# HiKapok/X-Detector

Hardware: AMD Instinct MI355X
Metric: images/sec at 480x480 Light-Head R-CNN, 1/2/4/8 MI355X + backbone MFMA util% (higher is better)
Workload: dtype f16x3 (split-precision f16 MFMA, f32 accumulate, f32 activations); 1 GPU; Full Light-Head R-CNN (Xception backbone + RPN + GPU proposals/NMS + PSROIAlign + light head + per-class NMS), 300 proposals, 480x480; batch_per_gpu=256, global_batch=256, image_size=480, concurrent_sub_batches=2, cross_terms=f16, input=whitened f32 [B,3,480,480] resident in HBM, parallelism=image-sharded dp1, weights=seeded random init (no checkpoint exists), graph_replay=True

## Files before the change

### x-detector_amd/csrc/common.h

```cpp
#pragma once
#include <hip/hip_runtime.h>
#include "../../include/xdet.h"
#include "conv_params.h"
#include "workspace.h"
#include <atomic>
#include <cstdint>
#include <cstdio>
#include <string>
#include <vector>

namespace xdet {

void set_last_error(const std::string& s);
int hip_fail(hipError_t e, const char* what, const char* file, int line);

#define XDET_HIP(expr)                                                          \
  do {                                                                          \
    hipError_t _e = (expr);                                                     \
    if (_e != hipSuccess) return ::xdet::hip_fail(_e, #expr, __FILE__, __LINE__); \
  } while (0)

#define XDET_LAUNCH_CHECK() XDET_HIP(hipGetLastError())

#define XDET_REQUIRE(cond, msg)                                   \
  do {                                                            \
    if (!(cond)) {                                                \
      ::xdet::set_last_error(std::string("invalid argument: ") + (msg)); \
      return XDET_ERR_INVALID_ARG;                        \
    }                                                             \
  } while (0)

#define XDET_TRY(expr)            \
  do {                            \
    int _rc = (expr);             \
    if (_rc != 0) return _rc;     \
  } while (0)

struct DeviceOnce {
  std::atomic<unsigned long long> done{0};
};
static inline int ensure_dynamic_lds(DeviceOnce& once, const void* kern, int bytes) {
  int dev = 0;
  XDET_HIP(hipGetDevice(&dev));
  const unsigned long long bit = 1ull << (dev & 63);
  if (once.done.load(std::memory_order_acquire) & bit) return XDET_OK;
  XDET_HIP(hipFuncSetAttribute(kern, hipFuncAttributeMaxDynamicSharedMemorySize, bytes));
  once.done.fetch_or(bit, std::memory_order_release);
  return XDET_OK;
}

static inline int round_up(int x, int m) { return (x + m - 1) / m * m; }
static inline int64_t cdiv(int64_t a, int64_t b) { return (a + b - 1) / b; }

int launch_conv_mfma_f32(const ConvParams& p, bool small_cin, int n_tile, hipStream_t s);
int launch_conv_mfma_split(const ConvParams& p, bool small_cin, int n_tile, int nsplit, hipStream_t s);
int launch_conv_mfma_dma(const ConvParams& p, int n_tile, int nsplit, hipStream_t s);
bool conv_dma_fold_applicable(const ConvParams& p, int n_tile, int nsplit);
int launch_conv_mfma_dma_fold(const ConvParams& p, hipStream_t s);
int64_t conv_ksplit_tiles(int64_t M, int cout_pad, int n_tile);
bool conv_ksplit_supported(int kh, int kw, int64_t n_pix_in, int ld_in, int cin_p, int cout_pad);
int launch_conv_mfma_ksplit(const ConvParams& p, int n_tile, int nsplit, int mode, int64_t scratch_tiles, hipStream_t s);
enum { PREC_F32 = 0, PREC_F16X3 = 1, PREC_F16 = 2 };

int launch_nchw_to_nhwc4(const float* in, float* out, int N, int C, int H, int W, int ldo, hipStream_t s);
int launch_depthwise3x3(const float* in, const float* w9c, float* out, int N, int H, int W, int C, int ld,
                        int dil, int relu_in, hipStream_t s);
int launch_maxpool3x3s2_add(const float* in, const float* res, float* out, int N, int H, int W, int C, int ld,
                            int Ho, int Wo, int pad_t, int pad_l, hipStream_t s);
int launch_maxpool3x3s2_bn_planes(const float* in, const float* scale, const float* shift, unsigned short* hi, unsigned short* lo,
                                  int N, int H, int W, int C, int ld, int Ho, int Wo, int pad_t, int pad_l, float mul,
                                  hipStream_t s, unsigned short* hi2 = nullptr, unsigned short* lo2 = nullptr, int c32_2 = 0,
                                  float mul2 = 1.f);
int launch_bn_relu(const float* in, const float* scale, const float* shift, float* out, unsigned short* hi, unsigned short* lo,
                   int64_t npix, int ld, float mul, hipStream_t s);
int launch_maxpool_v3s2_add(const float* in_hpooled, const float* res, float* out, int N, int H, int Wo, int C, int ld,
                            int Ho, int pad_t, hipStream_t s, unsigned short* sub_hi = nullptr, unsigned short* sub_lo = nullptr,
                            float sub_mul = 1.f);
int launch_range_check(const float* x, int N, size_t per_image, float limit, int* bad_per_image, hipStream_t s,
                       int groups = 1, size_t group_elems = 0, int relu = 0);
int launch_range_check_planes(const unsigned short* hi, int N, int64_t pix_per_image, int ld, int* bad_per_image,
                              hipStream_t s, int groups = 1, int64_t group_pix = 0);
int launch_relu_copy(const float* in, float* out, int64_t n, hipStream_t s);
int launch_stem_conv3x3s2(const float* in_nchw, const float* w27x32, const float* scale, const float* shift,
                          unsigned short* hi, unsigned short* lo, int N, int S, hipStream_t s);
int launch_split_f32(const float* in, unsigned short* hi, unsigned short* lo, int64_t n_pix, int ld, int relu,
                     hipStream_t s, float mul = 1.f, int x8 = 0, int x8_exp = 0);
int launch_planes_copy_blocks(const unsigned short* shi, const unsigned short* slo, unsigned short* dhi, unsigned short* dlo,
                              int64_t n_pix, int ld_src, int c32_dst, float r, hipStream_t s);
int launch_split_f32_subsample2(const float* in, unsigned short* hi, unsigned short* lo, int N, int H, int W, int ld,
                                hipStream_t s, const float* scale = nullptr, const float* shift = nullptr, float mul = 1.f,
                                int c32_dst = 0);
int launch_absmax_planes(const unsigned short* hi, int64_t n_halves, unsigned* out, hipStream_t s);
int launch_absmax_f32(const float* x, int64_t n, int relu, unsigned* out, hipStream_t s);
int launch_depthwise3x3_split(const float* in, const float* w9c, unsigned short* hi, unsigned short* lo, int N,
                              int H, int W, int C, int ld, int dil, int relu_in, hipStream_t s, int x8 = 0, int x8_exp = 0);

bool spectral_supported(int F);
int spectral_points(int F);
void spectral_tables(int F, std::vector<float>* fwd, std::vector<float>* inv);
void spectral_weights(const float* w, int T, int cin, int cout, int cin_ld, int cout_ld, int F, std::vector<float>* out);
int launch_dft_fwd(const float* in, int F, int ld, int axis, int N, int m_pad, const float* tab, unsigned short* hi,
                   unsigned short* lo, hipStream_t s);
int launch_dft_inv(const float* Y, int F, int ldn, int C_ld, int N, int m_pad, const float* tab, const float* scale,
                   const float* shift, int relu, float* out, int ldo, int axis, hipStream_t s);

bool sepconv_fused_supported(int cin_ld, int cout_pad, int dil);
int launch_sepconv_fused(const float* in, const float* w9c, const unsigned short* wt_hi_blocked,
                         const unsigned short* wt_lo_blocked, const float* scale, const float* shift, float* out, int N,
                         int H, int W, int ld, int ldo, int cout_pad, int relu_in, int relu_out, hipStream_t s,
                         int pool_pad_l = -1);

bool conv3x3_patch_supported(int kh, int kw, int cin, int cout_pad, int stride, int dil, int pad_mode);
int launch_conv3x3_patch(const unsigned short* in_hi, const unsigned short* in_lo, const unsigned short* wt_hi_blocked,
                         const unsigned short* wt_lo_blocked, const float* scale, const float* shift, float* out, int N, int H,
                         int W, int ldo, int relu, hipStream_t s);

bool resnet_stem7x7_supported(int kh, int kw, int cin, int cout, int stride, int pad_mode, int pad, int S);
int launch_resnet_stem7x7(const float* img_nchw, const unsigned short* wt_hi, const unsigned short* wt_lo, const float* scale,
                          const float* shift, float* out, int N, int S, hipStream_t s);

bool resnet_preconv_supported(int cin, int cmid, int64_t M);
int launch_resnet_preconv(const float* x, const float* pre_sc, const float* pre_sh, const unsigned short* w_hi,
                          const unsigned short* w_lo, const float* sc, const float* sh, unsigned short* out_hi,
                          unsigned short* out_lo, int64_t M, int cin, int cmid, hipStream_t s);

struct BneckLaunch {
  const float* x;
  const float *pre_sc, *pre_sh;
  const unsigned short *wa_hi, *wa_lo, *wb_hi, *wb_lo, *wc_hi, *wc_lo;
  const float *sc_a, *sh_a, *sc_b, *sh_b, *sc_c, *sh_c;
  const float *pl_sc, *pl_sh;
  float* out;
  unsigned short *out_hi, *out_lo;
  int H, W, cin, cmid, cout;
};
bool resnet_bneck_supported(int cin, int cmid, int cout, int H, int W, int N);
int launch_resnet_bneck(const BneckLaunch& a, int N, hipStream_t s);

int launch_preprocess_eval(const unsigned char* img, int H, int W, float* out_chw, int S, hipStream_t s);
int launch_preprocess_batch(const unsigned char* packed, int64_t packed_bytes, const int64_t* offsets,
                            const int* image_shapes, int N, int S, int mode, float* out_nchw, float* bbox_img,
                            hipStream_t s);

size_t preprocess_train_workspace_bytes(int N, int G);
int launch_preprocess_train(const unsigned char* packed, int64_t packed_bytes, const int64_t* offsets,
                            const int* image_shapes, const int* glabels, const float* gbboxes, const int* n_gt,
                            const int* image_ids, int N, int G, int S, unsigned seed, float* out_nchw, int* out_glabels,
                            float* out_gbboxes, int* out_n_gt, void* records, void* workspace, hipStream_t s);

int launch_psroialign(const float* feat, const float* rois, float* pooled, int32_t* index, int N, int C, int H,
                      int W, int R, int gw, int gh, int use_max, int layout, int ldc, int out_ld,
                      int rois_are_corners, hipStream_t s);
int launch_psroialign_grad(const float* rois, const float* grad_pooled, const int32_t* pooled_index, float* grad_out,
                           int N, int C, int H, int W, int R, int gw, int gh, int use_max, int layout, int ldc,
                           hipStream_t s);
int launch_psroialign_grad_ordered(const float* rois, const float* grad_pooled, int ld_grad, const int32_t* pooled_index,
                                   int ld_index, float* grad_out, int N, int C, int H, int W, int R, int gw, int gh,
                                   int use_max, int layout, int ldc, int corners, hipStream_t s);
int psroi_nhwc_scratch(const float* feat, int N, int C, int H, int W, hipStream_t s, float** scratch);

int launch_rotated_psroialign(const float* feat, const float* rois, const int32_t* orders, float* pooled,
                              int32_t* index, int N, int C, int H, int W, int R, int gw, int gh, int use_max,
                              int layout, int ldc, hipStream_t s);
int launch_rotated_psroialign_grad(const float* rois, const int32_t* orders, const float* grad_pooled,
                                   const int32_t* pooled_index, float* grad_out, int N, int C, int H, int W, int R,
                                   int gw, int gh, int use_max, int layout, int ldc, hipStream_t s);

struct ProposalWorkspace {
  unsigned long long* keys;
  float* cboxes;
  int* ranks;
  int* counts;
  float* sboxes;
  float* sscores;
  unsigned long long* cand;
  int* hist;
  int* bad;
  int* tbin;
  int* kept;
  unsigned* nms_ctl;
  unsigned long long* nms_sup;
// ... 23 lines not shown
```

### x-detector_amd/csrc/conv_mfma_dma.hip

```cpp
#include "common.h"
#include "conv_epilogue.h"
#include <cstdlib>
#include <cstring>
#include <type_traits>

namespace xdet {

#if CD_PROBE_LEVEL == 1
unsigned long long* g_conv_dma_probe = nullptr;
int g_conv_dma_probe_no_walk = 0;
#endif

typedef float f32x16 __attribute__((ext_vector_type(16)));
typedef _Float16 f16x8 __attribute__((ext_vector_type(8)));
typedef int x8frag __attribute__((ext_vector_type(8)));
typedef int x8half __attribute__((ext_vector_type(4)));
typedef unsigned short u16;

#define XDET_GLDS16(gptr, lptr)                                                                        \
  __builtin_amdgcn_global_load_lds((const __attribute__((address_space(1))) void*)(gptr),              \
                                   (__attribute__((address_space(3))) void*)(lptr), 16, 0, 0)

#ifndef CD_PROBE_LEVEL
#define CD_PROBE_LEVEL 0
#endif
#if CD_PROBE_LEVEL == 1
#define CD_PROBE_PARAM , unsigned long long* dbg
#define CD_PROBE_ARG , g_conv_dma_probe
#define CD_STAMP(vblk, slot)                                                      \
  do {                                                                            \
    if (dbg && threadIdx.x == 0) {                                                \
      dbg[((size_t)(vblk) * 5 + (slot)) * 2] = __builtin_amdgcn_s_memrealtime();  \
      dbg[((size_t)(vblk) * 5 + (slot)) * 2 + 1] = __builtin_amdgcn_s_memtime();  \
    }                                                                             \
  } while (0)
#define CD_STAMP_DRAINED(vblk, slot)                        \
  do {                                                      \
    asm volatile("s_waitcnt vmcnt(0)" ::: "memory");        \
    CD_STAMP(vblk, slot);                                   \
  } while (0)
#else
#define CD_PROBE_PARAM
#define CD_PROBE_ARG
#define CD_STAMP(vblk, slot) do {} while (0)
#define CD_STAMP_DRAINED(vblk, slot) do {} while (0)
#endif

constexpr int conv_dma_lds_bytes(int bm, int bn, int waves_m, int waves_n, bool walk) {
  const int stage = (2 * bm + 2 * bn) * 32 * 2;
  const int staging = waves_m * waves_n * 32 * (bn / waves_n + 4) * 4;
  return walk && stage + staging > 2 * stage ? stage + staging : 2 * stage;
}

template <int BM, int BN, int WAVES_M, int WAVES_N, int NSPLIT, int NSTAGE, bool PW = false, bool FOLD = false, bool X8 = false,
          bool GBUF = false, bool WALK = false>
__global__ __launch_bounds__(64 * WAVES_M * WAVES_N) void conv_dma_f16_kernel(ConvParams p_in, int nvb CD_PROBE_PARAM) {
  static_assert(NSTAGE == 2, "two LDS stages");
  static_assert(!(GBUF && PW), "GBUF is the buffer form of the NON-pointwise layers");
  static_assert(!X8 || (PW && NSPLIT == 3 && !FOLD), "x8: pointwise f16x3 layers only");
  static_assert(!WALK || ((PW || GBUF) && !FOLD), "the tile walk: the buffer forms (their weights are aimed per tile through a resource)");
  constexpr int NW = WAVES_M * WAVES_N;
  constexpr int WM = BM / WAVES_M, WN = BN / WAVES_N;
  constexpr int TM = WM / 32, TN = WN / 32;
  constexpr int A_IT = BM / (16 * NW);
  constexpr int B_IT = BN / (16 * NW);
  static_assert(A_IT >= 1 && B_IT >= 1, "tile too small for the wave count");
  constexpr int ROWB = 32;
  constexpr int STAGE = (2 * BM + 2 * BN) * ROWB;
  constexpr int EP_OFF = WALK ? STAGE : 0;
  constexpr int EP_BYTES = conv_dma_lds_bytes(BM, BN, WAVES_M, WAVES_N, WALK) - EP_OFF * 2;
  static_assert(conv_dma_lds_bytes(BM, BN, WAVES_M, WAVES_N, WALK) <= 160 * 1024, "stages + epilogue staging must fit a CU's LDS");

  extern __shared__ __attribute__((aligned(16))) u16 smem16[];

  const int tid = threadIdx.x;
  const int lane = tid & 63;
  const int wave = __builtin_amdgcn_readfirstlane(tid >> 6);
  const int wm = wave / WAVES_N, wn = wave % WAVES_N;
  const int nby = p_in.Cout_pad / BN;
  ConvParams p = p_in;
  auto tile_of = [&](int vb, int& tm0, int& tn0, int& tg) -> bool {
    const int slot = vb >> 3;
    if (p_in.group_rows) {
      const int mt = p_in.group_rows / BM;
      const int tpg = mt * nby;
      const int g = (slot / tpg) * 8 + (vb & 7);
      const int w = slot - (slot / tpg) * tpg;
      if ((int64_t)g * p_in.group_rows >= p_in.M) return false;
      if (p_in.group_live_rows && (w / nby) * BM >= p_in.group_live_rows) return false;
      tm0 = (g * mt + w / nby) * BM;
      tn0 = (w % nby) * BN;
      tg = g;
    } else {
      const int bx = (slot / nby) * 8 + (vb & 7);
      if (bx * BM >= p_in.M) return false;
      tm0 = bx * BM;
      tn0 = (slot % nby) * BN;
      tg = 0;
    }
    return true;
  };
  int vb = blockIdx.x;
  int m0, n0, grp;
  if constexpr (WALK) {
    while (vb < nvb && !tile_of(vb, m0, n0, grp)) vb += gridDim.x;
    if (vb >= nvb) return;
  } else {
    if (!tile_of(vb, m0, n0, grp)) return;
  }
  if (!WALK && p_in.group_rows) {
    p.wt_hi = p_in.wt_hi + (size_t)grp * p_in.group_wt_stride;
    p.wt_lo = p_in.wt_lo ? p_in.wt_lo + (size_t)grp * p_in.group_wt_stride : nullptr;
    p.scale = p_in.scale + (size_t)grp * p_in.Cout_pad;
    p.shift = p_in.shift + (size_t)grp * p_in.Cout_pad;
  }
  CD_STAMP(vb, 0);

  int iy0[A_IT], ix0[A_IT], pbase[A_IT], achunk[A_IT];
  size_t boff[B_IT];
  const int nk = p.Kp / 32;
  const int ntaps = p.KH * p.KW;
  const unsigned c32n = (unsigned)(p.ldi >> 5);

  __amdgpu_buffer_rsrc_t r_ah, r_al, r_bh, r_bl;
  unsigned a_vo[A_IT], b_vo[B_IT];
  int g_cc = 0, g_ky = 0, g_kx = 0, g_tap = 0;
  if (PW || GBUF) {
    const unsigned a_bytes = GBUF ? (unsigned)(((size_t)(((size_t)p.N * p.H * p.W + 15) >> 4) * c32n) << 10)
                                  : (unsigned)(((size_t)((p.M + 15) >> 4) * c32n) << 10);
    r_ah = __builtin_amdgcn_make_buffer_rsrc(const_cast<u16*>(p.in_hi), 0, (int)a_bytes, 0x00020000);
    r_al = __builtin_amdgcn_make_buffer_rsrc(const_cast<u16*>(NSPLIT > 1 ? p.in_lo : p.in_hi), 0, (int)a_bytes, 0x00020000);
  }
  auto aim = [&](int ln, int tm0, int tn0, int tg) {
    const int lr = ln >> 2;
    const int pos = ln & 3;
#pragma unroll
    for (int q = 0; q < A_IT; ++q) {
      const int rt = (wave * A_IT + q) * 16 + lr;
      achunk[q] = (pos ^ ((rt >> 2) & 3)) * 8;
      const int m = tm0 + rt;
      if (!PW) {
        if (m < p.M) {
          int hw = p.Ho * p.Wo, wo = p.Wo;
          if (WALK) asm volatile("" : "+s"(hw), "+s"(wo));
          const int n = m / hw;
          const int rem = m - n * hw;
          const int oy = rem / wo;
          const int ox = rem - oy * wo;
          iy0[q] = oy * p.stride - p.pad_t;
          ix0[q] = ox * p.stride - p.pad_l;
          pbase[q] = n * p.H * p.W;
        } else {
          iy0[q] = -(1 << 20);
          ix0[q] = 0;
          pbase[q] = 0;
        }
      } else {
        a_vo[q] = m < p.M ? (((unsigned)(m >> 4) * c32n) << 10) + (unsigned)((((m & 15) << 5) + achunk[q]) * 2) : 0xffffffffu;
      }
    }
#pragma unroll
    for (int q = 0; q < B_IT; ++q) {
      const int rt = (wave * B_IT + q) * 16 + lr;
      boff[q] = (size_t)(tn0 + rt) * 32 + (pos ^ ((rt >> 2) & 3)) * 8;
      if (PW || GBUF) b_vo[q] = (unsigned)(boff[q] * 2);
    }
    if (PW || GBUF) {
      const size_t wo = WALK ? (size_t)tg * p_in.group_wt_stride : 0;
      const unsigned b_bytes = (unsigned)((size_t)nk * p.Cout_pad * 64);
      r_bh = __builtin_amdgcn_make_buffer_rsrc(const_cast<u16*>(p.wt_hi + wo), 0, (int)b_bytes, 0x00020000);
      r_bl = __builtin_amdgcn_make_buffer_rsrc(const_cast<u16*>((NSPLIT > 1 ? p.wt_lo : p.wt_hi) + wo), 0, (int)b_bytes, 0x00020000);
    }
// ... 515 lines not shown
        }
      }
#pragma unroll
      for (int ks = 0; ks < 2; ++ks) {
        if (NSPLIT > 1) {
#pragma unroll
          for (int j = 0; j < TN; ++j) acc[0][j] = __builtin_amdgcn_mfma_f32_32x32x16_f16(al[ks], bh[ks][j], acc[0][j], 0, 0, 0);
#pragma unroll
          for (int j = 0; j < TN; ++j) acc[0][j] = __builtin_amdgcn_mfma_f32_32x32x16_f16(ah[ks], bl[ks][j], acc[0][j], 0, 0, 0);
        }
#pragma unroll
        for (int j = 0; j < TN; ++j) acc[0][j] = __builtin_amdgcn_mfma_f32_32x32x16_f16(ah[ks], bh[ks][j], acc[0][j], 0, 0, 0);
      }
    }
    ring = ring + PAIR >= NSTAGE ? ring + PAIR - NSTAGE : ring + PAIR;
  }
  asm volatile("s_waitcnt vmcnt(0)" ::: "memory");
  if (m0 + BM <= p.M) conv_epilogue_full<32, 32 * TN, 1, TN, NW, NSTAGE * STAGE * 2>(p, acc, smem16, wave, lane, WT ? (wave >> 1) : wave, WT ? (wave & 1) : 0, m0, n0);
  else conv_epilogue<32, 32 * TN, 1, TN, NW, NSTAGE * STAGE * 2>(p, acc, smem16, wave, lane, WT ? (wave >> 1) : wave, WT ? (wave & 1) : 0, m0, n0);
}

static bool pw_eligible(const ConvParams& p) {
  if (p.KH != 1 || p.KW != 1 || p.stride != 1 || p.pad_t != 0 || p.pad_l != 0 || p.H != p.Ho || p.W != p.Wo) return false;
  const size_t a_bytes = ((size_t)((p.M + 15) >> 4) * (size_t)(p.ldi >> 5)) << 10;
  const size_t b_bytes = (size_t)(p.Kp / 32) * p.Cout_pad * 64;
  return a_bytes < ((size_t)1 << 32) && b_bytes < ((size_t)1 << 32) && p.Cin_p == p.Kp;
}

template <int NSPLIT, bool PW = false, bool W8 = false, bool H64 = false>
static int launch_deep(const ConvParams& p, hipStream_t s) {
  if (!PW && pw_eligible(p)) return launch_deep<NSPLIT, true, W8, H64>(p, s);
  if constexpr (!W8 && !H64 && NSPLIT == 3) {
    if (!p.group_rows && cdiv(p.M, 128) * (p.Cout_pad / 64) <= 128) return launch_deep<NSPLIT, PW, false, true>(p, s);
    return launch_deep<NSPLIT, PW, true>(p, s);
  }
  constexpr int BM = H64 ? 64 : 128;
  constexpr size_t lds = (size_t)6 * (2 * BM + 2 * 64) * 32 * sizeof(u16);
  auto kern = conv_dma_deep_kernel<NSPLIT, PW, W8, H64>;
  static DeviceOnce once;
  XDET_TRY(ensure_dynamic_lds(once, reinterpret_cast<const void*>(kern), (int)lds));
  dim3 grid((unsigned)(cdiv(cdiv(p.M, BM), 8) * 8 * (p.Cout_pad / 64)));
  if (p.group_rows) {
    const int64_t groups = p.M / p.group_rows, tpg = (int64_t)(p.group_rows / BM) * (p.Cout_pad / 64);
    grid = dim3((unsigned)(cdiv(groups, 8) * 8 * tpg));
  }
  hipLaunchKernelGGL(kern, grid, dim3(W8 ? 512 : 256), lds, s, p);
  XDET_LAUNCH_CHECK();
  return XDET_OK;
}

static bool gbuf_eligible(const ConvParams& p) {
  if (p.group_rows != 0) return false;
  const size_t a_bytes = ((((size_t)p.N * p.H * p.W + 15) >> 4) * (size_t)(p.ldi >> 5)) << 10;
  const size_t b_bytes = (size_t)(p.Kp / 32) * p.Cout_pad * 64;
  return a_bytes < ((size_t)1 << 32) && b_bytes < ((size_t)1 << 32) && p.Kp == p.Cin_p * p.KH * p.KW;
}

static int device_cu_count(int* n_out) {
  static std::atomic<int> cus[64];
  int dev = 0;
  XDET_HIP(hipGetDevice(&dev));
  int n = cus[dev & 63].load(std::memory_order_acquire);
  if (n <= 0) {
    XDET_HIP(hipDeviceGetAttribute(&n, hipDeviceAttributeMultiprocessorCount, dev));
    cus[dev & 63].store(n, std::memory_order_release);
  }
  *n_out = n;
  return XDET_OK;
}

template <int BM, int BN, int WAVES_M, int WAVES_N, int NSPLIT, int NSTAGE = 2, bool PW = false, bool X8 = false, bool GBUF = false>
static int launch_d(const ConvParams& p, hipStream_t s) {
  if (!PW && pw_eligible(p)) return launch_d<BM, BN, WAVES_M, WAVES_N, NSPLIT, NSTAGE, true>(p, s);
  if constexpr (PW && !X8 && NSPLIT == 3) {
    if (p.x8) return launch_d<BM, BN, WAVES_M, WAVES_N, NSPLIT, NSTAGE, true, true>(p, s);
  }
  XDET_REQUIRE(X8 || !p.x8, "conv(dma): x8 planes need a pointwise f16x3 layer below 4 GiB");
  constexpr size_t lds = conv_dma_lds_bytes(BM, BN, WAVES_M, WAVES_N, false);
  if constexpr (!PW && !X8 && !GBUF && BM == 256 && BN == 256) {
    if (gbuf_eligible(p)) return launch_d<BM, BN, WAVES_M, WAVES_N, NSPLIT, NSTAGE, false, false, true>(p, s);
  }
  int64_t nvb = cdiv(cdiv(p.M, BM), 8) * 8 * (p.Cout_pad / BN);
  if (p.group_rows) {
    const int64_t groups = p.M / p.group_rows, tpg = (int64_t)(p.group_rows / BM) * (p.Cout_pad / BN);
    nvb = cdiv(groups, 8) * 8 * tpg;
  }
  if constexpr (BM == 256 && BN == 256 && (PW || GBUF)) {
    int cus = 0;
    XDET_TRY(device_cu_count(&cus));
    const int64_t wgs = cus / 8 * 8;
    bool walk = wgs >= 8 && nvb > wgs;
#if CD_PROBE_LEVEL == 1
    if (g_conv_dma_probe_no_walk) walk = false;
#endif
    if (walk) {
      constexpr size_t lds_w = conv_dma_lds_bytes(BM, BN, WAVES_M, WAVES_N, true);
      auto kern_w = conv_dma_f16_kernel<BM, BN, WAVES_M, WAVES_N, NSPLIT, NSTAGE, PW, false, X8, GBUF, true>;
      static DeviceOnce once_w;
      XDET_TRY(ensure_dynamic_lds(once_w, reinterpret_cast<const void*>(kern_w), (int)lds_w));
      hipLaunchKernelGGL(kern_w, dim3((unsigned)wgs), dim3(64 * WAVES_M * WAVES_N), lds_w, s, p, (int)nvb CD_PROBE_ARG);
      XDET_LAUNCH_CHECK();
      return XDET_OK;
    }
  }
  auto kern = conv_dma_f16_kernel<BM, BN, WAVES_M, WAVES_N, NSPLIT, NSTAGE, PW, false, X8, GBUF>;
  static DeviceOnce once;
  XDET_TRY(ensure_dynamic_lds(once, reinterpret_cast<const void*>(kern), (int)lds));
  hipLaunchKernelGGL(kern, dim3((unsigned)nvb), dim3(64 * WAVES_M * WAVES_N), lds, s, p, (int)nvb CD_PROBE_ARG);
  XDET_LAUNCH_CHECK();
  return XDET_OK;
}

bool conv_dma_fold_applicable(const ConvParams& p, int n_tile, int nsplit) {
  return n_tile == 128 && nsplit == 3 && p.group_rows == 0 && p.ksplit > 1 && cdiv(p.M, 256) * (p.Cout_pad / 128) >= 170;
}
int launch_conv_mfma_dma_fold(const ConvParams& p, hipStream_t s) {
  constexpr size_t lds = (size_t)2 * (2 * 256 + 2 * 128) * 32 * sizeof(u16);
  auto kern = conv_dma_f16_kernel<256, 128, 4, 2, 3, 2, false, true>;
  static DeviceOnce once;
  XDET_TRY(ensure_dynamic_lds(once, reinterpret_cast<const void*>(kern), (int)lds));
  dim3 grid((unsigned)(cdiv(cdiv(p.M, 256), 8) * 8 * (p.Cout_pad / 128)));
  hipLaunchKernelGGL(kern, grid, dim3(512), lds, s, p, (int)grid.x CD_PROBE_ARG);
  XDET_LAUNCH_CHECK();
  return XDET_OK;
}

int launch_conv_mfma_dma(const ConvParams& p_in, int n_tile, int nsplit, hipStream_t s) {
  ConvParams p = p_in;
  p.skip_dead = 1;
  XDET_REQUIRE(p.Kp % 32 == 0 && p.Cin_p % 32 == 0 && p.ldi >= p.Cin_p && p.ldi % 8 == 0,
               "conv(dma): channel counts must be padded to 32");
  XDET_REQUIRE(p.Cout_pad % n_tile == 0, "conv(dma): Cout_pad must be a multiple of the N tile");
  XDET_REQUIRE(p.in_hi && (nsplit == 1 || p.in_lo) && p.wt_hi && (nsplit == 1 || p.wt_lo) && p.zeros,
               "conv(dma): split planes missing");
  if (p.M <= 0) return XDET_OK;
  if (n_tile == 128 && nsplit == 3) {
    const int64_t b256 = cdiv(p.M, 256) * (p.Cout_pad / 256);
    const int nk = p.Kp / 32;
    int tile = 0;
    const bool full_rounds = b256 >= 240 && (b256 % 256 == 0 || b256 % 256 >= 240);
    if (p.Cout_pad % 256 == 0 && (b256 >= 512 || full_rounds || (b256 >= 200 && nk >= 40))) tile = 2;
    if (p.group_rows && p.group_rows % 256 != 0) tile = 0;
    if (tile == 2) return launch_d<256, 256, 2, 4, 3>(p, s);
  }
  if (n_tile == 128 && nsplit == 3 && !p.group_rows && !p.x8) {
    const int64_t b128 = cdiv(p.M, 128) * (p.Cout_pad / 128);
    if (b128 > 128 && b128 <= 256 && p.Kp / 32 >= 16 && p.Kp == p.Cin_p * p.KH * p.KW && p.ldi % 32 == 0 &&
        conv_ksplit_supported(p.KH, p.KW, (int64_t)p.N * p.H * p.W, p.ldi, p.Cin_p, p.Cout_pad)) {
      ConvParams q = p;
      q.ksplit = 1;
      q.ks_partial = nullptr;
      return launch_conv_mfma_ksplit(q, 128, 3, 2, 0, s);
    }
  }
  if (n_tile == 128 && nsplit == 3 && p.group_rows && p.group_rows % 64 == 0 && !p.x8) {
    const int live = p.group_live_rows ? p.group_live_rows : p.group_rows;
    const int64_t groups = p.M / p.group_rows, wgs = groups * cdiv(live, 64) * (p.Cout_pad / 64);
    if (live <= 64 && wgs <= 768) return launch_deep<3, false, false, true>(p, s);
  }
  if (n_tile == 128) {
    const int64_t b128 = cdiv(p.M, 128) * (p.Cout_pad / 128);
    if (nsplit == 3 && b128 <= 128 && (!p.group_rows || p.group_rows % 128 == 0)) {
      return p.x8 ? launch_d<128, 64, 4, 1, 3>(p, s) : launch_deep<3>(p, s);
    }
    return nsplit == 1 ? launch_d<128, 128, 2, 2, 1>(p, s) : launch_d<128, 128, 2, 2, 3>(p, s);
  }
  if (n_tile == 64) return nsplit == 1 ? launch_d<128, 64, 4, 1, 1>(p, s) : launch_d<128, 64, 4, 1, 3>(p, s);
  set_last_error("conv(dma): unsupported N tile");
// ... 5 lines not shown
```

### x-detector_amd/csrc/layers.h

```cpp
#pragma once
#include "common.h"
#include "device_mem.h"

#include <algorithm>
#include <cmath>
#include <cstring>
#include <vector>

namespace xdet {

struct Pow2Scaled {
  std::vector<float> host;
  float* dev = nullptr;
  int upload(int e, size_t n = 0) const {
    std::vector<float> v(std::max(n, host.size()), 0.f);
    for (size_t i = 0; i < host.size(); ++i) v[i] = ldexpf(host[i], e);
    XDET_HIP(hipMemcpy(dev, v.data(), v.size() * sizeof(float), hipMemcpyHostToDevice));
    return XDET_OK;
  }
};

extern int g_default_precision;

__host__ __device__ static inline unsigned short f32_to_f16_rne(float f) {
// ... 198 lines not shown
          hi[gc * kp + k] = h;
          if (precision == PREC_F16X3) lo[gc * kp + k] = f32_to_f16_rne(wv - f16_to_f32(h));
        }
        sc[gc] = ldexpf(sc[gc], -sh_k);
      }
      std::vector<float>().swap(wt);
      if (groups == 1) {
        XDET_TRY(d_wt_hi.upload(hi.data(), hi.size()));
        if (precision == PREC_F16X3) XDET_TRY(d_wt_lo.upload(lo.data(), lo.size()));
      }
      if (!small_cin) {
        std::vector<unsigned short> blk(hi.size());
        auto kblock = [&](const std::vector<unsigned short>& src) {
          for (size_t g = 0; g < G; ++g)
            for (int co = 0; co < cout_pad; ++co) {
              const unsigned short* r = &src[(g * cout_pad + co) * kp];
              for (int k = 0; k < kp; ++k) blk[g * mat + ((size_t)(k >> 5) * cout_pad + co) * 32 + (k & 31)] = r[k];
            }
        };
        kblock(hi);
        XDET_TRY(d_wt_hi_b.upload(blk.data(), blk.size()));
        if (precision == PREC_F16X3) {
          kblock(lo);
          XDET_TRY(d_wt_lo_b.upload(blk.data(), blk.size()));
          if (kh == 1 && kw == 1 && stride == 1 && groups == 1) {
            unsigned char* b8 = reinterpret_cast<unsigned char*>(blk.data());
            for (int co = 0; co < cout_pad; ++co)
              for (int k = 0; k < kp; ++k) {
                unsigned char* rec = b8 + ((size_t)(k >> 5) * cout_pad + co) * 64;
                rec[k & 31] = f32_to_e4m3(std::ldexp(f16_to_f32(lo[(size_t)co * kp + k]), 9));
                rec[32 + (k & 31)] = f32_to_e4m3(std::ldexp(f16_to_f32(hi[(size_t)co * kp + k]), -2));
              }
            XDET_TRY(d_wt_x8_b.upload(blk.data(), blk.size()));
          }
        }
      }
    }
    XDET_TRY(d_scale.upload(sc.data(), sc.size()));
    XDET_TRY(d_shift.upload(sh.data(), sh.size()));
    in_scale.host = sc;
    in_scale.dev = d_scale;
    return XDET_OK;
  }

  void out_shape(int H, int W, int* Ho, int* Wo, int* pt, int* pl) const {
    if (pad_mode == 1) {
      same_pad(H, kh, stride, dil, pt, Ho);
      same_pad(W, kw, stride, dil, pl, Wo);
    } else {
      *pt = pad_mode == 2 ? pad_t : 0;
      *pl = pad_mode == 2 ? pad_l : 0;
      const int tot_h = pad_mode == 2 ? (kh - 1) * dil : 0, tot_w = pad_mode == 2 ? (kw - 1) * dil : 0;
      *Ho = (H + tot_h - ((kh - 1) * dil + 1)) / stride + 1;
      *Wo = (W + tot_w - ((kw - 1) * dil + 1)) / stride + 1;
    }
  }
  int ld_in() const { return small_cin ? 4 : round_up(cin, 32); }
  int ld_out() const { return round_up(cout, 32); }
  double flops(int H, int W) const {
    int Ho, Wo, a, b;
    out_shape(H, W, &Ho, &Wo, &a, &b);
    return 2.0 * Ho * Wo * (double)cin * cout * kh * kw;
  }

  int forward(const ConvIO& io, int N, int H, int W, int ldi, int ldo, hipStream_t s) const {
    XDET_REQUIRE(ldi == ld_in(), "conv: ld_in must be round_up(cin,32) (4 for cin<=4)");
    XDET_REQUIRE(ldo == ld_out(), "conv: ld_out must be round_up(cout,32)");
    ConvParams p;
    p.in = io.in; p.wt = d_wt; p.wt_hi = d_wt_hi; p.wt_lo = d_wt_lo; p.out = io.out; p.scale = d_scale; p.shift = d_shift; p.res = io.res;
    p.N = N; p.H = H; p.W = W; p.ldi = ldi; p.ldo = ldo; p.ldr = ldo;
    out_shape(H, W, &p.Ho, &p.Wo, &p.pad_t, &p.pad_l);
    XDET_REQUIRE(p.Ho > 0 && p.Wo > 0, "conv: empty output");
    p.Cin_p = cin_p; p.Kp = kp; p.Cout_pad = cout_pad;
    p.KH = kh; p.KW = kw; p.stride = stride; p.dil = dil;
    p.M = N * p.Ho * p.Wo;
    p.relu_in = io.relu_in; p.relu_out = relu_out;
    p.in_hi = io.in_hi; p.in_lo = io.in_lo; p.zeros = io.zeros;
    p.out_hi = precision == PREC_F32 ? nullptr : io.out_hi; p.out_lo = io.out_lo; p.planes_relu = io.planes_relu;
    p.pl_scale = io.pl_scale; p.pl_shift = io.pl_shift; p.pl_c32 = pl_c32;
    p.group_rows = 0; p.group_wt_stride = 0;
    if (groups > 1) {
      XDET_REQUIRE(io.in_hi && io.group_rows > 0 && io.group_rows % 128 == 0 && (int64_t)io.group_rows * groups == p.M,
                   "conv(grouped): M must be groups * group_rows, group_rows a multiple of 128, input as planes");
      p.group_rows = io.group_rows;
      p.group_wt_stride = (long long)cout_pad * kp;
      p.group_live_rows = io.group_live_rows;
    }
    if (precision == PREC_F32) return launch_conv_mfma_f32(p, small_cin, n_tile, s);
    if (io.in_hi) {
      XDET_REQUIRE(!small_cin && io.relu_in == 0, "conv(dma): needs >= 32 input channels and no ReLU-on-load");
      p.wt_hi = d_wt_hi_b; p.wt_lo = d_wt_lo_b;
      if (io.x8) {
        XDET_REQUIRE(d_wt_x8_b && precision == PREC_F16X3 && ksplit < 1, "conv: x8 planes need a pointwise f16x3 layer without a split-K");
        p.wt_lo = d_wt_x8_b; p.x8 = 1; p.x8_exp = io.x8_exp;
      }
      if (ksplit >= 1 && groups == 1) {
        if (!conv_ksplit_supported(kh, kw, (int64_t)N * H * W, ldi, cin_p, cout_pad)) {
          if (ksplit == 1 && !ks_narrow) return launch_conv_mfma_dma(p, n_tile, precision == PREC_F16X3 ? 3 : 1, s);
          XDET_REQUIRE(ksplit == 1, "conv(ksplit): this batch's planes or weights exceed the split-K kernel's 4 GiB addressing (or the "
                                    "filter is not 1x1 / 3x3); a split reduction cannot change kernel family: run smaller batches");
          return launch_conv_mfma_dma(p, 64, precision == PREC_F16X3 ? 3 : 1, s);
        }
        p.ksplit = ksplit; p.ks_partial = d_ks_partial; p.ks_ticket = d_ks_ticket;
        return launch_conv_mfma_ksplit(p, cout_pad % 128 == 0 && !ks_narrow ? 128 : 64, precision == PREC_F16X3 ? 3 : 1, ks_mode, ks_tiles, s);
      }
      return launch_conv_mfma_dma(p, n_tile, precision == PREC_F16X3 ? 3 : 1, s);
    }
    return launch_conv_mfma_split(p, small_cin, n_tile, precision == PREC_F16X3 ? 3 : 1, s);
  }
  bool dma_capable() const { return precision != PREC_F32 && !small_cin; }
};

struct SpectralConv : LayerBase {
  int F = 0, NB = 0, axis = 0, cin = 0, cin_ld = 0, cout = 0, cout_ld = 0, relu = 0;
  ConvLayer G;
  Pow2Scaled tab_fwd;
  DevMem<float> d_tf, d_ti, d_scale, d_shift;
  static int m_pad(int F, int N) { return N * F <= 128 ? 128 : round_up(N * F, 256); }
  int m_pad(int N) const { return m_pad(F, N); }
  size_t planes_halves(int N) const { return (size_t)NB * m_pad(N) * 2 * cin_ld; }
  size_t y_floats(int N) const { return (size_t)NB * m_pad(N) * 2 * cout_ld; }
  int init(const float* w, int T, int cin_, int cout_, int axis_, int F_, const float* scale, const float* shift, int relu_) {
    XDET_REQUIRE(w && T > 0 && T % 2 == 1 && T <= 15 && cin_ > 0 && cout_ > 0 && (axis_ == 0 || axis_ == 1),
                 "spectral conv: an odd number of taps (<= 15) along axis 0 | 1");
    XDET_REQUIRE(spectral_supported(F_), "spectral conv: the feature-map side must be 16, 30 or 50");
    XDET_REQUIRE(g_default_precision != PREC_F32, "spectral conv: needs a split-precision mode");
    kind = 3;
    F = F_; NB = spectral_points(F) / 2; axis = axis_; relu = relu_;
    cin = cin_; cin_ld = round_up(cin, 32); cout = cout_; cout_ld = round_up(cout, 32);
    {
      std::vector<float> wb;
      spectral_weights(w, T, cin, cout, cin_ld, cout_ld, F, &wb);
      XDET_TRY(G.init(1, 1, 2 * cin_ld, 2 * cout_ld, 1, 1, 0, 0, 0, wb.data(), nullptr, nullptr, 0, NB));
    }
    device = G.device;
    std::vector<float> ti, sc(cout_ld, 0.f), sh(cout_ld, 0.f);
    spectral_tables(F, &tab_fwd.host, &ti);
    for (int c = 0; c < cout; ++c) { sc[c] = scale ? scale[c] : 1.f; sh[c] = shift ? shift[c] : 0.f; }
    XDET_TRY(d_tf.upload(tab_fwd.host.data(), tab_fwd.host.size()));
    XDET_TRY(d_ti.upload(ti.data(), ti.size()));
    XDET_TRY(d_scale.upload(sc.data(), sc.size()));
    XDET_TRY(d_shift.upload(sh.data(), sh.size()));
    tab_fwd.dev = d_tf;
    return XDET_OK;
  }
  int set_in_exp(int e) {
    XDET_TRY(tab_fwd.upload(-e));
    return G.set_in_exp(e);
  }
  int dft_fwd(const float* in, int N, unsigned short* x_hi, unsigned short* x_lo, hipStream_t s) const {
    return launch_dft_fwd(in, F, cin_ld, axis, N, m_pad(N), d_tf, x_hi, x_lo, s);
  }
  int gemm(int N, const unsigned short* x_hi, const unsigned short* x_lo, float* y, hipStream_t s) const {
    ConvIO io;
    io.in_hi = x_hi; io.in_lo = x_lo; io.zeros = G.d_zeros; io.out = y;
    io.group_rows = m_pad(N); io.group_live_rows = N * F;
    return G.forward(io, 1, 1, NB * m_pad(N), 2 * cin_ld, 2 * cout_ld, s);
  }
  int dft_inv(int N, const float* y, float* out, int ldo, hipStream_t s) const {
    return launch_dft_inv(y, F, 2 * cout_ld, cout_ld, N, m_pad(N), d_ti, d_scale, d_shift, relu, out, ldo, axis, s);
  }
  int forward(const float* in, int N, unsigned short* x_hi, unsigned short* x_lo, float* y, float* out, int ldo,
              hipStream_t s) const {
    XDET_TRY(dft_fwd(in, N, x_hi, x_lo, s));
    XDET_TRY(gemm(N, x_hi, x_lo, y, s));
    return dft_inv(N, y, out, ldo, s);
  }
};

struct DepthwiseLayer : LayerBase {
  int C, dil, ld;
  DevMem<float> d_w;
  Pow2Scaled taps;
  int out_exp = 0;
  bool host_stale = false;
  int set_kernel_device(const float* k33c1, hipStream_t s);
  int set_out_exp(int e) {
    XDET_REQUIRE(!host_stale, "depthwise: the kernel was refreshed on the device (xdet_depthwise_set_kernel_device): the host "
                              "copy of the taps is stale, an activation exponent cannot be applied");
    XDET_TRY(taps.upload(-e));
    out_exp = e;
    return XDET_OK;
  }
  int init(int C_, int dil_, const float* w33c1) {
    XDET_REQUIRE(C_ > 0 && dil_ > 0 && w33c1, "depthwise: bad arguments");
    kind = 2;
    XDET_HIP(hipGetDevice(&device));
    C = C_; dil = dil_; ld = round_up(C, 32);
    std::vector<float> w((size_t)9 * ld, 0.f);
    for (int t = 0; t < 9; ++t)
      for (int c = 0; c < C; ++c) w[(size_t)t * ld + c] = w33c1[(size_t)t * C + c];
    XDET_TRY(d_w.upload(w.data(), w.size()));
    taps.host = w;
    taps.dev = d_w;
    return XDET_OK;
  }
  int forward(const float* in, int N, int H, int W, int ld_, float* out, int relu_in, hipStream_t s) const {
    XDET_REQUIRE(ld_ == ld, "depthwise: ld must be round_up(C,32)");
    return launch_depthwise3x3(in, d_w, out, N, H, W, C, ld, dil, relu_in, s);
  }
};

}
```

### x-detector_amd/csrc/spectral.hip

```cpp
#include "common.h"
#include "cu_prims.h"

#include <cmath>
#include <vector>

namespace xdet {

__device__ __forceinline__ size_t sp_blocked_off(size_t pix, int c, int c32n) {
  return (((pix >> 4) * (size_t)c32n + (size_t)(c >> 5)) << 9) + ((pix & 15) << 5) + (size_t)(c & 31);
}

__device__ __forceinline__ void sp_store_split(u16* __restrict__ hi, u16* __restrict__ lo, size_t off, const float4 v) {
  const _Float16 h0 = (_Float16)v.x, h1 = (_Float16)v.y, h2 = (_Float16)v.z, h3 = (_Float16)v.w;
  f16x4 hv = {h0, h1, h2, h3};
  f16x4 lv = {(_Float16)(v.x - (float)h0), (_Float16)(v.y - (float)h1), (_Float16)(v.z - (float)h2),
              (_Float16)(v.w - (float)h3)};
  *reinterpret_cast<uint2*>(hi + off) = *reinterpret_cast<uint2*>(&hv);
  *reinterpret_cast<uint2*>(lo + off) = *reinterpret_cast<uint2*>(&lv);
}

template <int F, int L>
__global__ __launch_bounds__(256) void dft_fwd_kernel(const float* __restrict__ in, int ld, int axis, int M, int m_pad,
                                                      const float* __restrict__ tab, u16* __restrict__ hi,
                                                      u16* __restrict__ lo) {
// ... 5 lines not shown
  const int c = cblk * 32 + (lane & 7) * 4;
  const int m = blockIdx.x * 8 + (lane >> 3);
  const bool ok = m < M;
  const int n = m / F, o = m - n * F;
  const float* base = in + ((size_t)n * F * F + (axis == 0 ? o : o * F)) * ld + c;
  const size_t step = (size_t)(axis == 0 ? F : 1) * ld;
  float4 v[F];
#pragma unroll
  for (int i = 0; i < F; ++i) v[i] = ok ? *reinterpret_cast<const float4*>(base + i * step) : make_float4(0.f, 0.f, 0.f, 0.f);
  const int c32n = (2 * ld) >> 5;
  const int nbz = (NB + (int)gridDim.z - 1) / (int)gridDim.z;
  const int b_lo = (int)blockIdx.z * nbz, b_hi = min(NB, b_lo + nbz);
#pragma unroll 1
  for (int b = b_lo; b < b_hi; ++b) {
    const float* __restrict__ tr = tab + (size_t)b * 2 * F;
    const float* __restrict__ ti = tr + F;
    float4 re = make_float4(0.f, 0.f, 0.f, 0.f), im = re;
#pragma unroll
    for (int i = 0; i < F; ++i) {
      const float cr = tr[i], ci = ti[i];
      re.x = fmaf(v[i].x, cr, re.x); re.y = fmaf(v[i].y, cr, re.y); re.z = fmaf(v[i].z, cr, re.z); re.w = fmaf(v[i].w, cr, re.w);
      im.x = fmaf(v[i].x, ci, im.x); im.y = fmaf(v[i].y, ci, im.y); im.z = fmaf(v[i].z, ci, im.z); im.w = fmaf(v[i].w, ci, im.w);
    }
    if (ok) {
      const size_t row = (size_t)b * m_pad + m;
      sp_store_split(hi, lo, sp_blocked_off(row, c, c32n), re);
      sp_store_split(hi, lo, sp_blocked_off(row, ld + c, c32n), im);
    }
  }
}

template <int F, int L, int ZI>
__global__ __launch_bounds__(256) void dft_inv_kernel(const float* __restrict__ Y, int ldn, int C_ld, int M, int m_pad,
                                                      const float* __restrict__ tab, const float* __restrict__ scale,
                                                      const float* __restrict__ shift, int relu, float* __restrict__ out,
                                                      int ldo, int axis) {
  constexpr int NB = L / 2;
  const int lane = threadIdx.x & 63;
  const int wave = __builtin_amdgcn_readfirstlane(threadIdx.x >> 6);
  const int cblk = blockIdx.y * 4 + wave;
  if (cblk * 32 >= C_ld) return;
  const int c = cblk * 32 + (lane & 7) * 4;
  const int m = blockIdx.x * 8 + (lane >> 3);
  if (m >= M) return;
  const int n = m / F, o = m - n * F;
  static_assert(F % ZI == 0, "output positions must divide evenly");
  constexpr int G = F / ZI;
  const int i0 = (int)blockIdx.z * G;
  float4 acc[G];
#pragma unroll
  for (int i = 0; i < G; ++i) acc[i] = make_float4(0.f, 0.f, 0.f, 0.f);
#pragma unroll 1
  for (int b = 0; b < NB; ++b) {
    const float* row = Y + ((size_t)b * m_pad + m) * ldn + c;
    const float4 yr = *reinterpret_cast<const float4*>(row);
    const float4 yi = *reinterpret_cast<const float4*>(row + C_ld);
    const float* __restrict__ tr = tab + (size_t)b * 2 * F + i0;
    const float* __restrict__ ti = tr + F;
#pragma unroll
    for (int i = 0; i < G; ++i) {
      const float cr = tr[i], ci = ti[i];
      acc[i].x = fmaf(yr.x, cr, acc[i].x); acc[i].y = fmaf(yr.y, cr, acc[i].y);
      acc[i].z = fmaf(yr.z, cr, acc[i].z); acc[i].w = fmaf(yr.w, cr, acc[i].w);
      acc[i].x = fmaf(yi.x, ci, acc[i].x); acc[i].y = fmaf(yi.y, ci, acc[i].y);
      acc[i].z = fmaf(yi.z, ci, acc[i].z); acc[i].w = fmaf(yi.w, ci, acc[i].w);
    }
  }
  const float4 sc = *reinterpret_cast<const float4*>(scale + c), sh = *reinterpret_cast<const float4*>(shift + c);
  const size_t step = (size_t)(axis == 0 ? F : 1) * ldo;
  float* base = out + ((size_t)n * F * F + (axis == 0 ? o : o * F)) * ldo + c + (size_t)i0 * step;
#pragma unroll
  for (int i = 0; i < G; ++i) {
    float4 t = make_float4(fmaf(acc[i].x, sc.x, sh.x), fmaf(acc[i].y, sc.y, sh.y), fmaf(acc[i].z, sc.z, sh.z),
                           fmaf(acc[i].w, sc.w, sh.w));
    if (relu) {
      t.x = (t.x > 0.f || t.x != t.x) ? t.x : 0.f; t.y = (t.y > 0.f || t.y != t.y) ? t.y : 0.f;
      t.z = (t.z > 0.f || t.z != t.z) ? t.z : 0.f; t.w = (t.w > 0.f || t.w != t.w) ? t.w : 0.f;
    }
    *reinterpret_cast<float4*>(base + i * step) = t;
  }
}

bool spectral_supported(int F) { return F == 16 || F == 30 || F == 50; }
int spectral_points(int F) { return F + 14; }

void spectral_tables(int F, std::vector<float>* fwd, std::vector<float>* inv) {
  const int L = spectral_points(F), NB = L / 2;
  fwd->assign((size_t)NB * 2 * F, 0.f);
  inv->assign((size_t)NB * 2 * F, 0.f);
  const double w = 2.0 * M_PI / L;
  for (int i = 0; i < F; ++i) {
    (*fwd)[(size_t)0 * 2 * F + i] = 1.f;
    (*fwd)[(size_t)0 * 2 * F + F + i] = (i & 1) ? -1.f : 1.f;
    (*inv)[(size_t)0 * 2 * F + i] = (float)(1.0 / L);
    (*inv)[(size_t)0 * 2 * F + F + i] = (float)(((i & 1) ? -1.0 : 1.0) / L);
    for (int b = 1; b < NB; ++b) {
      const double th = w * (double)(((long long)b * i) % L);
      (*fwd)[((size_t)b * 2) * F + i] = (float)std::cos(th);
      (*fwd)[((size_t)b * 2 + 1) * F + i] = (float)(-std::sin(th));
      (*inv)[((size_t)b * 2) * F + i] = (float)(2.0 * std::cos(th) / L);
      (*inv)[((size_t)b * 2 + 1) * F + i] = (float)(-2.0 * std::sin(th) / L);
    }
  }
}

void spectral_weights(const float* w, int T, int cin, int cout, int cin_ld, int cout_ld, int F, std::vector<float>* out) {
  const int L = spectral_points(F), NB = L / 2, pad = T / 2;
  const size_t K2 = 2 * (size_t)cin_ld, N2 = 2 * (size_t)cout_ld;
  out->assign((size_t)NB * K2 * N2, 0.f);
  const double om = 2.0 * M_PI / L;
  std::vector<double> cr(T), ci(T);
  std::vector<double> gr(cout), gi(cout);
  for (int b = 0; b < NB; ++b) {
    float* B = out->data() + (size_t)b * K2 * N2;
    if (b == 0) {
      for (int k = 0; k < cin; ++k) {
        for (int n = 0; n < cout; ++n) { gr[n] = 0; gi[n] = 0; }
        for (int t = 0; t < T; ++t) {
          const int j = ((pad - t) % L + L) % L;
          const double sgn = (j & 1) ? -1.0 : 1.0;
          const float* src = w + ((size_t)t * cin + k) * cout;
          for (int n = 0; n < cout; ++n) { gr[n] += src[n]; gi[n] += sgn * src[n]; }
        }
        float* r0 = B + (size_t)k * N2;
        float* r1 = B + ((size_t)cin_ld + k) * N2;
        for (int n = 0; n < cout; ++n) { r0[n] = (float)gr[n]; r1[cout_ld + n] = (float)gi[n]; }
      }
      continue;
    }
    for (int t = 0; t < T; ++t) {
      const int j = ((pad - t) % L + L) % L;
      const double th = om * (double)(((long long)b * j) % L);
      cr[t] = std::cos(th);
      ci[t] = -std::sin(th);
    }
    for (int k = 0; k < cin; ++k) {
      for (int n = 0; n < cout; ++n) { gr[n] = 0; gi[n] = 0; }
      for (int t = 0; t < T; ++t) {
        const float* src = w + ((size_t)t * cin + k) * cout;
        const double a = cr[t], bb = ci[t];
        for (int n = 0; n < cout; ++n) { gr[n] += a * src[n]; gi[n] += bb * src[n]; }
      }
      float* r0 = B + (size_t)k * N2;
      float* r1 = B + ((size_t)cin_ld + k) * N2;
      for (int n = 0; n < cout; ++n) {
        r0[n] = (float)gr[n]; r0[cout_ld + n] = (float)gi[n];
        r1[n] = (float)(-gi[n]); r1[cout_ld + n] = (float)gr[n];
      }
    }
  }
}

template <int F>
static int launch_fwd_t(const float* in, int ld, int axis, int N, int m_pad, const float* tab, u16* hi, u16* lo, hipStream_t s) {
  const int M = N * F;
  const int64_t wgs = cdiv(M, 8) * cdiv(ld / 32, 4);
  const unsigned z = wgs >= 512 ? 1u : wgs >= 256 ? 2u : wgs >= 128 ? 4u : 6u;
  dim3 grid((unsigned)cdiv(M, 8), (unsigned)cdiv(ld / 32, 4), z);
  hipLaunchKernelGGL((dft_fwd_kernel<F, F + 14>), grid, dim3(256), 0, s, in, ld, axis, M, m_pad, tab, hi, lo);
  XDET_LAUNCH_CHECK();
  return XDET_OK;
}
template <int F>
static int launch_inv_t(const float* Y, int ldn, int C_ld, int N, int m_pad, const float* tab, const float* scale,
                        const float* shift, int relu, float* out, int ldo, int axis, hipStream_t s) {
  const int M = N * F;
  if (cdiv(M, 8) * cdiv(C_ld / 32, 4) < 256) {
    dim3 grid((unsigned)cdiv(M, 8), (unsigned)cdiv(C_ld / 32, 4), 2);
    hipLaunchKernelGGL((dft_inv_kernel<F, F + 14, 2>), grid, dim3(256), 0, s, Y, ldn, C_ld, M, m_pad, tab, scale, shift, relu,
                       out, ldo, axis);
  } else {
    dim3 grid((unsigned)cdiv(M, 8), (unsigned)cdiv(C_ld / 32, 4));
    hipLaunchKernelGGL((dft_inv_kernel<F, F + 14, 1>), grid, dim3(256), 0, s, Y, ldn, C_ld, M, m_pad, tab, scale, shift, relu,
                       out, ldo, axis);
  }
  XDET_LAUNCH_CHECK();
  return XDET_OK;
}

int launch_dft_fwd(const float* in, int F, int ld, int axis, int N, int m_pad, const float* tab, unsigned short* hi,
                   unsigned short* lo, hipStream_t s) {
  XDET_REQUIRE(ld % 32 == 0 && (axis == 0 || axis == 1) && N > 0 && m_pad >= N * F, "dft_fwd: bad arguments");
  switch (F) {
    case 16: return launch_fwd_t<16>(in, ld, axis, N, m_pad, tab, hi, lo, s);
    case 30: return launch_fwd_t<30>(in, ld, axis, N, m_pad, tab, hi, lo, s);
    case 50: return launch_fwd_t<50>(in, ld, axis, N, m_pad, tab, hi, lo, s);
  }
  set_last_error("dft_fwd: unsupported feature-map side");
  return XDET_ERR_UNSUPPORTED;
}

int launch_dft_inv(const float* Y, int F, int ldn, int C_ld, int N, int m_pad, const float* tab, const float* scale,
                   const float* shift, int relu, float* out, int ldo, int axis, hipStream_t s) {
  XDET_REQUIRE(C_ld % 32 == 0 && ldn >= 2 * C_ld && ldo >= C_ld && (axis == 0 || axis == 1) && N > 0 && m_pad >= N * F,
               "dft_inv: bad arguments");
  switch (F) {
    case 16: return launch_inv_t<16>(Y, ldn, C_ld, N, m_pad, tab, scale, shift, relu, out, ldo, axis, s);
    case 30: return launch_inv_t<30>(Y, ldn, C_ld, N, m_pad, tab, scale, shift, relu, out, ldo, axis, s);
    case 50: return launch_inv_t<50>(Y, ldn, C_ld, N, m_pad, tab, scale, shift, relu, out, ldo, axis, s);
  }
  set_last_error("dft_inv: unsupported feature-map side");
  return XDET_ERR_UNSUPPORTED;
}

}
```

Baseline: 4092 images/sec.

## Shrink spectral DFT length and compact grouped-conv tile grid to live rows

The spectral conv transform length is reduced from F+14 to roughly F+8, rounded to even. Only the 'same' outputs are kept, so circular wraparound only needs half the tap span, and the shorter length means fewer frequency bins in the forward DFT, the per-bin GEMM and the inverse DFT. Separately, the grouped-conv tile walker now counts tiles only over the live rows of each group and maps virtual blocks onto that compacted space. Blocks are no longer launched just to exit on dead padded rows. The risk is that the tighter DFT length relies on an aliasing argument for the zero-padded halo, and the new block-to-tile mapping changes how tiles are interleaved across XCDs.

```diff
diff --git a/x-detector_amd/csrc/common.h b/x-detector_amd/csrc/common.h
--- a/x-detector_amd/csrc/common.h
+++ b/x-detector_amd/csrc/common.h
@@ -96,7 +96,8 @@
                               int H, int W, int C, int ld, int dil, int relu_in, hipStream_t s, int x8 = 0, int x8_exp = 0);
 
 bool spectral_supported(int F);
-int spectral_points(int F);
+constexpr int kSpectralMaxTaps = 15;
+constexpr int spectral_points(int F) { return (F + kSpectralMaxTaps / 2 + 1) / 2 * 2; }
 void spectral_tables(int F, std::vector<float>* fwd, std::vector<float>* inv);
 void spectral_weights(const float* w, int T, int cin, int cout, int cin_ld, int cout_ld, int F, std::vector<float>* out);
 int launch_dft_fwd(const float* in, int F, int ld, int axis, int N, int m_pad, const float* tab, unsigned short* hi,
diff --git a/x-detector_amd/csrc/conv_mfma_dma.hip b/x-detector_amd/csrc/conv_mfma_dma.hip
--- a/x-detector_amd/csrc/conv_mfma_dma.hip
+++ b/x-detector_amd/csrc/conv_mfma_dma.hip
@@ -83,11 +83,13 @@
     const int slot = vb >> 3;
     if (p_in.group_rows) {
       const int mt = p_in.group_rows / BM;
-      const int tpg = mt * nby;
-      const int g = (slot / tpg) * 8 + (vb & 7);
-      const int w = slot - (slot / tpg) * tpg;
-      if ((int64_t)g * p_in.group_rows >= p_in.M) return false;
-      if (p_in.group_live_rows && (w / nby) * BM >= p_in.group_live_rows) return false;
+      const int live = p_in.group_live_rows ? p_in.group_live_rows : p_in.group_rows;
+      const int tpg = ((live + BM - 1) / BM) * nby;
+      const int q = nvb >> 3;
+      const int t = (vb & 7) * q + slot;
+      if (slot >= q || t >= (p_in.M / p_in.group_rows) * tpg) return false;
+      const int g = t / tpg;
+      const int w = t - g * tpg;
       tm0 = (g * mt + w / nby) * BM;
       tn0 = (w % nby) * BN;
       tg = g;
@@ -769,8 +771,9 @@
   }
   int64_t nvb = cdiv(cdiv(p.M, BM), 8) * 8 * (p.Cout_pad / BN);
   if (p.group_rows) {
-    const int64_t groups = p.M / p.group_rows, tpg = (int64_t)(p.group_rows / BM) * (p.Cout_pad / BN);
-    nvb = cdiv(groups, 8) * 8 * tpg;
+    const int64_t live = p.group_live_rows ? p.group_live_rows : p.group_rows;
+    const int64_t groups = p.M / p.group_rows, tpg = cdiv(live, BM) * (p.Cout_pad / BN);
+    nvb = cdiv(groups * tpg, 8) * 8;
   }
   if constexpr (BM == 256 && BN == 256 && (PW || GBUF)) {
     int cus = 0;
diff --git a/x-detector_amd/csrc/layers.h b/x-detector_amd/csrc/layers.h
--- a/x-detector_amd/csrc/layers.h
+++ b/x-detector_amd/csrc/layers.h
@@ -304,6 +304,7 @@
     if (groups > 1) {
       XDET_REQUIRE(io.in_hi && io.group_rows > 0 && io.group_rows % 128 == 0 && (int64_t)io.group_rows * groups == p.M,
                    "conv(grouped): M must be groups * group_rows, group_rows a multiple of 128, input as planes");
+      XDET_REQUIRE(io.group_live_rows >= 0 && io.group_live_rows <= io.group_rows, "conv(grouped): live rows beyond the group");
       p.group_rows = io.group_rows;
       p.group_wt_stride = (long long)cout_pad * kp;
       p.group_live_rows = io.group_live_rows;
@@ -343,7 +344,7 @@
   size_t planes_halves(int N) const { return (size_t)NB * m_pad(N) * 2 * cin_ld; }
   size_t y_floats(int N) const { return (size_t)NB * m_pad(N) * 2 * cout_ld; }
   int init(const float* w, int T, int cin_, int cout_, int axis_, int F_, const float* scale, const float* shift, int relu_) {
-    XDET_REQUIRE(w && T > 0 && T % 2 == 1 && T <= 15 && cin_ > 0 && cout_ > 0 && (axis_ == 0 || axis_ == 1),
+    XDET_REQUIRE(w && T > 0 && T % 2 == 1 && T <= kSpectralMaxTaps && cin_ > 0 && cout_ > 0 && (axis_ == 0 || axis_ == 1),
                  "spectral conv: an odd number of taps (<= 15) along axis 0 | 1");
     XDET_REQUIRE(spectral_supported(F_), "spectral conv: the feature-map side must be 16, 30 or 50");
     XDET_REQUIRE(g_default_precision != PREC_F32, "spectral conv: needs a split-precision mode");
diff --git a/x-detector_amd/csrc/spectral.hip b/x-detector_amd/csrc/spectral.hip
--- a/x-detector_amd/csrc/spectral.hip
+++ b/x-detector_amd/csrc/spectral.hip
@@ -111,7 +111,6 @@
 }
 
 bool spectral_supported(int F) { return F == 16 || F == 30 || F == 50; }
-int spectral_points(int F) { return F + 14; }
 
 void spectral_tables(int F, std::vector<float>* fwd, std::vector<float>* inv) {
   const int L = spectral_points(F), NB = L / 2;
@@ -186,7 +185,7 @@
   const int64_t wgs = cdiv(M, 8) * cdiv(ld / 32, 4);
   const unsigned z = wgs >= 512 ? 1u : wgs >= 256 ? 2u : wgs >= 128 ? 4u : 6u;
   dim3 grid((unsigned)cdiv(M, 8), (unsigned)cdiv(ld / 32, 4), z);
-  hipLaunchKernelGGL((dft_fwd_kernel<F, F + 14>), grid, dim3(256), 0, s, in, ld, axis, M, m_pad, tab, hi, lo);
+  hipLaunchKernelGGL((dft_fwd_kernel<F, spectral_points(F)>), grid, dim3(256), 0, s, in, ld, axis, M, m_pad, tab, hi, lo);
   XDET_LAUNCH_CHECK();
   return XDET_OK;
 }
@@ -196,11 +195,11 @@
   const int M = N * F;
   if (cdiv(M, 8) * cdiv(C_ld / 32, 4) < 256) {
     dim3 grid((unsigned)cdiv(M, 8), (unsigned)cdiv(C_ld / 32, 4), 2);
-    hipLaunchKernelGGL((dft_inv_kernel<F, F + 14, 2>), grid, dim3(256), 0, s, Y, ldn, C_ld, M, m_pad, tab, scale, shift, relu,
+    hipLaunchKernelGGL((dft_inv_kernel<F, spectral_points(F), 2>), grid, dim3(256), 0, s, Y, ldn, C_ld, M, m_pad, tab, scale, shift, relu,
                        out, ldo, axis);
   } else {
     dim3 grid((unsigned)cdiv(M, 8), (unsigned)cdiv(C_ld / 32, 4));
-    hipLaunchKernelGGL((dft_inv_kernel<F, F + 14, 1>), grid, dim3(256), 0, s, Y, ldn, C_ld, M, m_pad, tab, scale, shift, relu,
+    hipLaunchKernelGGL((dft_inv_kernel<F, spectral_points(F), 1>), grid, dim3(256), 0, s, Y, ldn, C_ld, M, m_pad, tab, scale, shift, relu,
                        out, ldo, axis);
   }
   XDET_LAUNCH_CHECK();
```

New measurement: 4151 images/sec, median of 6. +1.4%, better.
